# MobilityFirst/gigapaxos

Measured on AMD Instinct MI355X. Metric: decided_ops_per_sec, higher is better.
Workload: dtype int32; 1 GPU; BASELINE config #3: 1000000 Paxos groups x 3 replicas per GPU, synthetic shuffled accept-reply stream; step = propose_batch(G) + accept_reply_batch(K*G votes), inputs resident in HBM; groups_per_gpu=1000000, groups_total=1000000, replicas=3, rounds_seeded_individually=96, ordered_proposals_promise=True, ordered_batches_mask=1, parallelism=groups sharded across GPUs, no collective on the decide path

## Files before the change

gigapaxos_amd/csrc/gpx_ar16.hip.h:

```cpp
#pragma once
#include "gpx_kernels.hip.h"
#include "gpx_tiles.hip.h"

struct __attribute__((aligned(16))) Vote16 {
  int32_t idx, slot, maxcp;
  uint32_t meta;
};
#define V16_LG_MASK 0x3fffu
#define V16_ESC 0x4000u
#define V16_MAX_SHIFT 10
#define GPX_TL_BUCKET_DYN_MAX (152 * 1024)

struct Stage16 {
  int32_t* base;
  int64_t n;
  __host__ __device__ __forceinline__ int32_t* gidx() const { return base; }
  __host__ __device__ __forceinline__ int32_t* slot() const { return base + n; }
  __host__ __device__ __forceinline__ int32_t* bnum() const { return base + 2 * n; }
  __host__ __device__ __forceinline__ int32_t* bcoord() const { return base + 3 * n; }
  __host__ __device__ __forceinline__ int32_t* median() const { return base + 4 * n; }
  __host__ __device__ __forceinline__ uint8_t* kind() const { return (uint8_t*)(base + 5 * n); }
};
struct VoteCols {
  const int32_t *bnum, *bcoord, *acceptor;
  const int32_t *slot, *maxcp;
};
struct PlaceCols {
  int32_t *gidx, *slot, *bnum, *bcoord, *median;
  uint8_t* kind;
  int32_t div;
  uint32_t mul;
  __device__ __forceinline__ int32_t quot(int32_t x) const { return div == 1 ? x : (int32_t)__umulhi((uint32_t)x, mul); }
};
#define GPX_IP_LEARN_WORD 8

__device__ __forceinline__ void put_vote16(const DevScratch& X, int32_t* lds, int32_t G, int32_t mask,
                                           int32_t b0n, int32_t b0c, int64_t i, int32_t g, int32_t slot,
                                           int32_t acc, int32_t maxcp, int32_t bn, int32_t bc) {
  if ((uint32_t)(g - X.g_base) >= (uint32_t)(X.g_end - X.g_base)) return;
  (void)G;
  const int32_t pos = bucket_take(lds, (g - X.g_base) >> X.shift);
  const bool esc = bn != b0n || bc != b0c || (uint32_t)acc > 0xffffu;
  Vote16 v;
  v.idx = (int32_t)i;
  v.slot = slot;
  v.maxcp = maxcp;
  v.meta = (uint32_t)(g & mask) | (esc ? V16_ESC : ((uint32_t)acc << 16));
  ((Vote16*)X.rec)[pos] = v;
}

template <bool VEC>
__global__ __launch_bounds__(GPX_FBLOCK) void k_scatter_ar16(
    int32_t n, int32_t ntiles, int32_t G, DevScratch X, const int32_t* __restrict__ gidx,
    const int32_t* __restrict__ bnum, const int32_t* __restrict__ bcoord,
    const int32_t* __restrict__ slot, const int32_t* __restrict__ acceptor,
    const int32_t* __restrict__ max_cp) {
  extern __shared__ int32_t lds[];
  const int32_t tile = tile_of_block(ntiles);
  if (tile >= ntiles) return;
  if (X.gate && *X.unsorted != X.epoch) return;
  const int32_t b0n = bnum[0], b0c = bcoord[0];
  scatter_init(X, tile, lds);
  const int64_t base = (int64_t)tile * GPX_TILE;
  const int32_t mask = X.gb - 1;
  if (VEC) {
#pragma unroll
    for (int j = 0; j < GPX_TILE_VECS; j++) {
      const int64_t i0 = base + (int64_t)(j * GPX_FBLOCK + threadIdx.x) * 4;
      if (i0 + 3 < n) {
        const I4 g4 = *(const I4*)(gidx + i0), s4 = *(const I4*)(slot + i0);
        const I4 a4 = *(const I4*)(acceptor + i0), m4 = *(const I4*)(max_cp + i0);
        const I4 n4 = *(const I4*)(bnum + i0), c4 = *(const I4*)(bcoord + i0);
        put_vote16(X, lds, G, mask, b0n, b0c, i0 + 0, g4.x, s4.x, a4.x, m4.x, n4.x, c4.x);
        put_vote16(X, lds, G, mask, b0n, b0c, i0 + 1, g4.y, s4.y, a4.y, m4.y, n4.y, c4.y);
        put_vote16(X, lds, G, mask, b0n, b0c, i0 + 2, g4.z, s4.z, a4.z, m4.z, n4.z, c4.z);
        put_vote16(X, lds, G, mask, b0n, b0c, i0 + 3, g4.w, s4.w, a4.w, m4.w, n4.w, c4.w);
      } else {
        for (int q = 0; q < 4; q++) {
          const int64_t i = i0 + q;
          if (i < n)
            put_vote16(X, lds, G, mask, b0n, b0c, i, gidx[i], slot[i], acceptor[i], max_cp[i], bnum[i],
                       bcoord[i]);
        }
      }
    }
  } else {
#pragma unroll
    for (int j = 0; j < GPX_TILE_ITEMS; j++) {
      const int64_t i = base + j * GPX_FBLOCK + threadIdx.x;
      if (i < n)
        put_vote16(X, lds, G, mask, b0n, b0c, i, gidx[i], slot[i], acceptor[i], max_cp[i], bnum[i],
                   bcoord[i]);
    }
  }
// ... 261 lines not shown
        have = true;
        el = el && sl == s0;
      }
      if (have) {
        const int32_t d = jsub(P.next, s0);
        el = el && d >= 1 && d <= S.W;
      }
    }
    fast = __all(el);
  }
  if (fast) {
    if (OP == B16_AR) {
      const int32_t G = S.G, k = (int32_t)GF_K(P.gf);
      int32_t mem[KMAX], ns[KMAX];
#pragma unroll
      for (int j = 0; j < KMAX; j++) {
        mem[j] = (j < k) ? P.mem[j] : 0;
        ns[j] = (j < k) ? P.ns[j] : 0;
      }
      const int64_t off = (int64_t)(s0 & (S.W - 1)) * G + g;
      const uint32_t e0 = (P.have_pe && s0 == jsub(P.next, 1)) ? P.pe : S.p_ring[off];
      uint32_t e = e0;
      int32_t pcount = P.pcount;
      bool ns_dirty = false;
      auto vote = [&](int32_t i, uint32_t p, int32_t acc, int32_t maxcp) {
        int32_t midx = -1;
#pragma unroll
        for (int q = 0; q < KMAX; q++) {
          if (q < k && mem[q] == acc) {
            midx = q;
            if (ns[q] < maxcp) {
              ns[q] = maxcp;
              ns_dirty = true;
            }
          }
        }
        if (e & PR_PRESENT) {
          if (midx >= 0) e |= (1u << midx);
          if (__popc(e & 0xffffu) > k / 2) {
            slotA[p] = s0;
            cpA[p] = median_minus<KMAX>(ns, k);
            metaA[p] = (uint32_t)GPX_D_DECISION;
            it.omask |= 1u << i;
            it.nout++;
            e = 0;
            pcount--;
          }
        }
      };
      if (!__any(esc)) {
        for (int32_t i = 0; i < nvote; i++) {
          const uint32_t p = (uint32_t)start + (uint32_t)pstride * (uint32_t)((it.order >> (4 * i)) & 15ull);
          vote(i, p, (int32_t)(metaA[p] >> 16), cpA[p]);
        }
      } else {
        for (int32_t i = 0; i < nvote; i++) {
          if ((skip >> i) & 1u) continue;
          const uint32_t p = (uint32_t)start + (uint32_t)pstride * (uint32_t)((it.order >> (4 * i)) & 15ull);
          const uint32_t meta = metaA[p];
          vote(i, p, (meta & V16_ESC) ? in.acceptor[idxA[p]] : (int32_t)(meta >> 16), cpA[p]);
        }
      }
      if (e != e0) S.p_ring[off] = e;
      if (ns_dirty) {
#pragma unroll
        for (int q = 0; q < KMAX; q++)
          if (q < k) S.node_slots[(int64_t)q * G + g] = ns[q];
      }
      if (pcount != P.pcount) S.c_pcount[g] = pcount;
    }
  } else {
    replay(it);
  }
}

struct TileLds {
  int32_t* pre;
  uint16_t* st;
};
#define GPX_TILE_LDS_DECL(TILES_)                                   \
  __shared__ int32_t s_pre_[(TILES_) ? GPX_TL_MAXWG + 1 : 1];       \
  __shared__ uint16_t s_st_[(TILES_) ? GPX_TL_MAXWG : 1];           \
  const TileLds TL{s_pre_, s_st_}
template <int OP, int KMAX, bool TILES = false>
__device__ __forceinline__ void bucket16_body(const DevState& S, const DevScratch& X, const Stage16& O, const VoteCols& in,
                                              const AcceptOut& R, uint8_t* __restrict__ status, const TileLds& TL,
                                              const TileArea& A = TileArea{}, int32_t b_in = -1,
                                              const PlaceCols& IP = PlaceCols{}) {
  extern __shared__ __attribute__((aligned(16))) int32_t lds[];
  constexpr bool AC = OP != B16_AR;
  if ((AC || X.gate) && *X.unsorted != X.epoch) return;
  int32_t b = b_in >= 0 ? b_in : (int32_t)blockIdx.x;
  if (TILES && A.xcd_rows && b_in < 0) {
    b = tile_of_block(X.nbk);
    if (b >= X.nbk) return;
  }
  const int32_t gb = X.gb;
  const int32_t l = (int32_t)threadIdx.x;
  int32_t boff, nb;
  int32_t* const s_pre = TL.pre;
  uint16_t* const s_st = TL.st;
  if (TILES) TL_STAMP(4096 + b, 0);
  if (TILES) {
    const unsigned long long* r0 = (const unsigned long long*)A.off + (uint32_t)(b >> 2) * (uint32_t)A.nwg_pad;
    const unsigned long long* r1 = (const unsigned long long*)A.off + (uint32_t)((b + 1) >> 2) * (uint32_t)A.nwg_pad;
    const int32_t per = (A.nwg + gb - 1) >> X.shift;
    int32_t cw[4], ssum = 0, csum = 0;
#pragma unroll
    for (int q = 0; q < 4; q++) {
      const int32_t w = l * per + q;
      cw[q] = 0;
      if (q < per && w < A.nwg) {
        const unsigned long long e0 = r0[w];
        const unsigned long long e1 = ((b & 3) == 3) ? r1[w] : e0;
        const uint16_t o0 = (uint16_t)(e0 >> (16 * (b & 3))), o1 = (uint16_t)(e1 >> (16 * ((b + 1) & 3)));
        const int32_t st = (int32_t)(o0 & 0x7fffu);
        cw[q] = (int32_t)(o1 & 0x7fffu) - st;
        s_st[w] = o0;
        ssum += st;
        csum += cw[q];
      }
    }
    int32_t ex = block_exscan_and_sum_rt(csum, ssum, &nb, &boff);
#pragma unroll
    for (int q = 0; q < 4; q++) {
      const int32_t w = l * per + q;
      if (q < per && w < A.nwg) {
        s_pre[w] = ex;
        ex += cw[q];
      }
    }
    if (l == 0) {
      s_pre[A.nwg] = nb;
      X.bucket_off[b] = boff;
      if (nb == 0) X.bucket_nout[b] = 0;
    }
  } else {
    boff = X.bucket_off[b];
    nb = X.bucket_off[b + 1] - boff;
    if (threadIdx.x == 0) {
      X.bucket_tot[b] = 0;
      if (nb == 0) X.bucket_nout[b] = 0;
    }
  }
  if (nb == 0) return;
  const int32_t g = X.g_base + (b << X.shift) + l;
#ifdef GPX_B16_NOPRELOAD
  const bool pre = false;
#else
  const bool pre = !AC && 2 * nb >= gb;
#endif
  CoordPre<KMAX> P;
  P.have_pe = false;
  P.my_bnum = P.my_bcoord = 0;
  if (pre && g < X.g_end) coord_preload<KMAX>(S, g, P);
  const int32_t L = X.lds_recs;
  int32_t* lcnt = lds;
  int32_t* lcur = lds + gb;
  int32_t* idxA = lds + 2 * gb;
  int32_t* slotA = idxA + L;
  int32_t* cpA = slotA + L;
  uint32_t* metaA = (uint32_t*)(cpA + L);
  const bool in_lds = nb <= L;
  Vote16* recG = (Vote16*)X.rec + boff;
  unsigned long long* keysG = X.perm + boff;
  lcnt[l] = 0;
  const int32_t slot0 = TILES ? A.ref[0] : 0;
  const int32_t ref_bn = TILES ? A.ref[1] : in.bnum[0], ref_bc = TILES ? A.ref[2] : in.bcoord[0];
  int32_t ip_pb = 0, ip_span = -1;
  if (TILES && !AC && IP.div) {
    ip_pb = IP.quot(boff);
    ip_span = IP.quot(boff + nb) - ip_pb;
  }
  int32_t srch = 0;
  if (TILES)
    while ((1 << srch) < A.nwg) srch++;
  auto tile_find = [&](int32_t j) -> int32_t {
    int32_t lo = 0, hi = A.nwg;
    for (int32_t t = 0; t < srch; t++) {
      const int32_t mid = (lo + hi) >> 1;
      const bool up = s_pre[mid] <= j;
      lo = up ? mid : lo;
      hi = up ? hi : mid;
    }
    return lo;
  };
  auto tile_adv = [&](int32_t j, int32_t lo) -> int32_t {
    while (s_pre[lo + 1] <= j) lo++;
    return lo;
  };
  auto tile_pos = [&](int32_t j, int32_t lo, uint32_t* wide) -> uint32_t {
    const uint32_t st = s_st[lo];
    *wide = st & TL_WIDE;
    return __umul24((uint32_t)lo, (uint32_t)A.tile) + (st & 0x7fffu) + (uint32_t)(j - s_pre[lo]);
  };
  auto tile_exp = [&](const Vote8 raw, uint32_t p, uint32_t wide, int32_t lo) -> Vote16 {
    const I4 x = tile_expand(raw, wide ? A.ext + p : (const int2*)nullptr, lo, A.tile, slot0, in.slot, in.maxcp);
    Vote16 v;
    v.idx = x.x, v.slot = x.y, v.maxcp = x.z, v.meta = (uint32_t)x.w;
    return v;
  };
  auto tile_at = [&](int32_t j, int32_t lo) -> Vote16 {
    uint32_t wide;
    const uint32_t p = tile_pos(j, lo, &wide);
    return tile_exp(A.recs[p], p, wide, lo);
  };
  auto tile_rec = [&](int32_t j) -> Vote16 { return tile_at(j, tile_find(j)); };
  if (TILES) __syncthreads();
  if (TILES) TL_STAMP(4096 + b, 1);
#ifdef GPX_ABL_STOP
  if (TILES && GPX_ABL_STOP == 1) return;
#endif
  if (TILES && !in_lds) {
    for (int32_t j = l; j < nb; j += gb) recG[j] = tile_rec(j);
    __threadfence_block();
  }
  __syncthreads();
  Vote16 r0, r1, r2, r3;
  r0.meta = r1.meta = r2.meta = r3.meta = 0;
  r0.idx = r1.idx = r2.idx = r3.idx = 0;
  r0.slot = r1.slot = r2.slot = r3.slot = 0;
  r0.maxcp = r1.maxcp = r2.maxcp = r3.maxcp = 0;
  const bool from_tiles = TILES && in_lds;
  const int32_t pl = from_tiles ? (nb + gb - 1) >> X.shift : 0;
  const int32_t jb = from_tiles ? l * pl : l, jstep = from_tiles ? 1 : gb;
  const int32_t jend = from_tiles ? min(jb + pl, nb) : nb;
  const bool v0 = jb < jend, v1 = jb + jstep < jend, v2 = jb + 2 * jstep < jend, v3 = jb + 3 * jstep < jend;
  int32_t lo3 = 0;
  if (from_tiles) {
    int32_t l0 = 0, l1 = 0, l2 = 0;
    uint32_t p0 = 0, p1 = 0, p2 = 0, p3 = 0, w0 = 0, w1 = 0, w2 = 0, w3 = 0;
    Vote8 q0{}, q1{}, q2{}, q3{};
    if (v0) lo3 = l0 = tile_find(jb), p0 = tile_pos(jb, l0, &w0), q0 = A.recs[p0];
    if (v1) lo3 = l1 = tile_adv(jb + 1, l0), p1 = tile_pos(jb + 1, l1, &w1), q1 = A.recs[p1];
    if (v2) lo3 = l2 = tile_adv(jb + 2, l1), p2 = tile_pos(jb + 2, l2, &w2), q2 = A.recs[p2];
    if (v3) lo3 = tile_adv(jb + 3, l2), p3 = tile_pos(jb + 3, lo3, &w3), q3 = A.recs[p3];
    if (v0) r0 = tile_exp(q0, p0, w0, l0);
    if (v1) r1 = tile_exp(q1, p1, w1, l1);
    if (v2) r2 = tile_exp(q2, p2, w2, l2);
    if (v3) r3 = tile_exp(q3, p3, w3, lo3);
  } else {
    if (v0) r0 = recG[jb];
    if (v1) r1 = recG[jb + jstep];
    if (v2) r2 = recG[jb + 2 * jstep];
    if (v3) r3 = recG[jb + 3 * jstep];
  }
  const int32_t tail0 = jb + 4 * jstep;
  auto for_tail = [&](auto&& f) {
    if (from_tiles) {
      int32_t lo = lo3;
      for (int32_t j = tail0; j < jend; j++) {
        lo = tile_adv(j, lo);
        f(tile_at(j, lo));
      }
    } else {
      for (int32_t j = tail0; j < jend; j += jstep) f(recG[j]);
    }
  };
  constexpr int KSLOT = KMAX <= 4 ? 4 : 8;
  bool slotted = false;
  if (TILES && !AC && in_lds && KSLOT * gb <= L) {
    bool over = false;
    auto put_row = [&](const Vote16& v) {
      const int32_t lg = (int32_t)(v.meta & V16_LG_MASK);
      const int32_t t = atomicAdd(&lcnt[lg], 1);
      if (t < KSLOT) {
        const int32_t p = t * gb + lg;
        idxA[p] = v.idx;
        slotA[p] = v.slot;
        cpA[p] = v.maxcp;
        metaA[p] = v.meta;
      } else {
        over = true;
      }
    };
    if (v0) put_row(r0);
    if (v1) put_row(r1);
    if (v2) put_row(r2);
    if (v3) put_row(r3);
    for_tail([&](const Vote16& v) { put_row(v); });
    slotted = !__syncthreads_or(over);
    if (!slotted) {
      lcnt[l] = 0;
      __syncthreads();
    }
  }
  int32_t c, start, any_long = 0;
  if (slotted) {
    c = lcnt[l];
    start = l;
    if (TILES) TL_STAMP(4096 + b, 3);
#ifdef GPX_ABL_STOP
    if (TILES && GPX_ABL_STOP == 2) return;
#endif
    if (pre && g < X.g_end) coord_preload_ring<KMAX>(S, g, P);
  } else {
  {
    if (v0) atomicAdd(&lcnt[r0.meta & V16_LG_MASK], 1);
    if (v1) atomicAdd(&lcnt[r1.meta & V16_LG_MASK], 1);
    if (v2) atomicAdd(&lcnt[r2.meta & V16_LG_MASK], 1);
// ... 132 lines not shown
    it.cur = 0;
    if (live) ar16_replay_group<OP, KMAX>(S, X, g, it, P, in, R, status, idxA, slotA, cpA, metaA, start, pstride, c);
    nout = it.nout;
    omask = it.omask;
    if (TILES) TL_STAMP(4096 + b, 4);
#ifdef GPX_ABL_STOP
    if (TILES && GPX_ABL_STOP == 3) return;
#endif
    int32_t tout;
    const int32_t ex = block_exscan_rt(nout, &tout);
    const int32_t pb = in_place(tout);
    for (int32_t q = 0; q < nout; q++) {
      int32_t sl, md, kd;
      it.output(q, &sl, &md, &kd, &omask);
      put((int64_t)boff + ex + q, sl, md, kd);
      if (pb >= 0) put_in_place(pb + ex + q, sl, md, kd);
    }
    if (l == 0) X.bucket_nout[b] = tout;
    if (TILES) TL_STAMP(4096 + b, 5);
  } else {
    VoteIter<false, AC> it;
    it.idxA = idxA;
    it.slotA = slotA;
    it.cpA = cpA;
    it.metaA = metaA;
    it.recG = recG;
    it.keys = keysG + start;
    it.in = in;
    it.b0n = ref_bn;
    it.b0c = ref_bc;
    it.start = start;
    it.stride = 1;
    it.c = c;
    it.done = 0;
    it.nout = 0;
    it.nib = false;
    it.order = 0;
    it.omask = 0;
    it.cur = 0;
    if (live) replay(it);
    nout = it.nout;
    int32_t tout;
    const int32_t ex = block_exscan_rt(nout, &tout);
    const int32_t pb = in_place(tout);
    for (int32_t q = 0; q < nout; q++) {
      int32_t sl, md, kd;
      it.output(q, &sl, &md, &kd, &omask);
      put((int64_t)boff + ex + q, sl, md, kd);
      if (pb >= 0) put_in_place(pb + ex + q, sl, md, kd);
    }
    if (l == 0) X.bucket_nout[b] = tout;
  }
}

template <int OP, int KMAX>
__global__ __launch_bounds__(1024) GPX_AR16_ATTR void k_bucket16(DevState S, DevScratch X, Stage16 O, VoteCols in,
                                                   AcceptOut R, uint8_t* __restrict__ status) {
  GPX_TILE_LDS_DECL(false);
  bucket16_body<OP, KMAX>(S, X, O, in, R, status, TL);
}
struct TilesKernArgs {
  DevState S;
  DevScratch X;
  Stage16 O;
  VoteCols in;
  uint8_t* status;
  TileArea A;
  PlaceCols IP;
};
static_assert(alignof(DevState) == 8 && alignof(DevScratch) == 8 && alignof(Stage16) == 8 && alignof(VoteCols) == 8 &&
                  alignof(TileArea) == 8 && alignof(PlaceCols) == 8,
              "kernarg layout");
static_assert(sizeof(DevState) % 8 == 0 && sizeof(DevScratch) % 8 == 0 && sizeof(Stage16) % 8 == 0 && sizeof(VoteCols) % 8 == 0 &&
                  sizeof(TileArea) % 8 == 0 && sizeof(PlaceCols) % 8 == 0,
              "kernarg layout");
#ifndef GPX_LAZY
#define GPX_LAZY 7
#endif
template <bool LAZY, class T>
__device__ __forceinline__ const T& lazy_pick(const T& from_kernarg, const T& by_value) {
  if constexpr (LAZY) return from_kernarg;
  else return by_value;
}
#define GPX_TILES_KERNEL_BODY(KM)                                                                                          \
  GPX_TILE_LDS_DECL(true);                                                                                                 \
  const TilesKernArgs* ka = (const TilesKernArgs*)__builtin_amdgcn_kernarg_segment_ptr();                                  \
  bucket16_body<B16_AR, KM, true>(lazy_pick<(GPX_LAZY & 16) != 0>(ka->S, S), lazy_pick<(GPX_LAZY & 2) != 0>(ka->X, X), O,  \
                                  lazy_pick<(GPX_LAZY & 1) != 0>(ka->in, in), AcceptOut{},                                 \
                                  (GPX_LAZY & 8) ? ka->status : status, TL, lazy_pick<(GPX_LAZY & 32) != 0>(ka->A, A), -1, \
                                  lazy_pick<(GPX_LAZY & 4) != 0>(ka->IP, IP))
template <int KMAX>
__global__ __launch_bounds__(1024) GPX_AR16_ATTR void k_bucket_ar16_tiles(DevState S, DevScratch X, Stage16 O, VoteCols in,
                                                                         uint8_t* __restrict__ status, TileArea A, PlaceCols IP) {
  GPX_TILES_KERNEL_BODY(KMAX);
}
#ifndef GPX_K4_WAVES
#define GPX_K4_WAVES 6
#endif
__global__ __launch_bounds__(1024) __attribute__((amdgpu_waves_per_eu(GPX_K4_WAVES, 8))) void k_bucket_ar16_tiles_k4(
    DevState S, DevScratch X, Stage16 O, VoteCols in, uint8_t* __restrict__ status, TileArea A, PlaceCols IP) {
  GPX_TILES_KERNEL_BODY(4);
}
__global__ __launch_bounds__(1024) __attribute__((amdgpu_waves_per_eu(6, 8))) void k_bucket_ar16_tiles_k5(
    DevState S, DevScratch X, Stage16 O, VoteCols in, uint8_t* __restrict__ status, TileArea A, PlaceCols IP) {
  GPX_TILES_KERNEL_BODY(5);
}
__global__ __launch_bounds__(1024) __attribute__((amdgpu_waves_per_eu(6, 8))) void k_bucket_ar16_k5(
    DevState S, DevScratch X, Stage16 O, VoteCols in, AcceptOut R, uint8_t* __restrict__ status) {
  GPX_TILE_LDS_DECL(false);
  bucket16_body<B16_AR, 5>(S, X, O, in, R, status, TL);
}

__global__ __launch_bounds__(GPX_BLOCK) void k_emit_dec16(
    DevScratch X, Stage16 O, int32_t* __restrict__ d_gidx, int32_t* __restrict__ d_slot,
    int32_t* __restrict__ d_bnum, int32_t* __restrict__ d_bcoord, int32_t* __restrict__ d_median,
    uint8_t* __restrict__ d_kind, int32_t* total_out, unsigned long long* acc, const int32_t* base_in,
    int32_t* chain_out, int32_t* in_place = nullptr, int32_t nvotes = 0, const int32_t* __restrict__ c_bnum = nullptr,
    const int32_t* __restrict__ c_bcoord = nullptr) {
  if (X.gate && *X.unsorted != X.epoch) return;
  const bool placed = in_place && in_place[3] != (int32_t)X.epoch;
  if (placed && blockIdx.x != gridDim.x - 1) return;
  const int32_t base0 = base_in ? *base_in : 0;
  const int32_t b = blockIdx.x;
  int32_t before = 0;
  for (int32_t t = threadIdx.x; t < b; t += GPX_BLOCK) before += X.bucket_nout[t];
  int32_t pre;
  block_exscan(before, &pre);
  const int32_t out0 = base0 + pre;
  if (b == (int32_t)gridDim.x - 1 && threadIdx.x == 0) {
    const int32_t tot = pre + X.bucket_nout[b];
    if (total_out) *total_out = base0 + tot;
    if (chain_out) *chain_out = base0 + tot;
    if (acc) atomicAdd(acc, (unsigned long long)tot);
    if (in_place && !placed && tot > 0 && nvotes % tot == 0 && nvotes / tot <= 64 && X.xabort)
      __hip_atomic_store(X.xabort + GPX_IP_LEARN_WORD, (uint32_t)(nvotes / tot), __ATOMIC_RELAXED, __HIP_MEMORY_SCOPE_SYSTEM);
    if (in_place) in_place[placed ? 5 : 6]++;
  }
  if (placed) return;
  const int32_t nd = X.bucket_nout[blockIdx.x];
  const int64_t src = X.bucket_off[blockIdx.x];
  if (threadIdx.x == 0) X.bucket_tot[blockIdx.x] = 0;
  for (int32_t t = threadIdx.x; t < nd; t += GPX_BLOCK) {
    const int32_t g = O.gidx()[src + t];
    d_gidx[out0 + t] = g;
    d_slot[out0 + t] = O.slot()[src + t];
    d_bnum[out0 + t] = c_bnum ? c_bnum[g] : O.bnum()[src + t];
    d_bcoord[out0 + t] = c_bnum ? c_bcoord[g] : O.bcoord()[src + t];
    d_median[out0 + t] = O.median()[src + t];
    d_kind[out0 + t] = O.kind()[src + t];
  }
}

__global__ __launch_bounds__(GPX_BLOCK) void k_emit_runs16(DevScratch X, Stage16 O, int32_t* __restrict__ x_gidx,
                                                          int32_t* __restrict__ x_first,
                                                          int32_t* __restrict__ x_count, int32_t* total_out) {
  if (*X.unsorted != X.epoch) return;
  const int32_t out0 = emit_base(X, total_out, nullptr);
  const int32_t nd = X.bucket_nout[blockIdx.x];
  const int64_t src = X.bucket_off[blockIdx.x];
  for (int32_t t = threadIdx.x; t < nd; t += GPX_BLOCK) {
    x_gidx[out0 + t] = O.gidx()[src + t];
    x_first[out0 + t] = O.slot()[src + t];
    x_count[out0 + t] = O.median()[src + t];
  }
}

__global__ __launch_bounds__(GPX_BLOCK) void k_unpack_replies(DevScratch X, int32_t n, const I4* __restrict__ rows,
                                                             int32_t* __restrict__ r_bnum,
                                                             int32_t* __restrict__ r_bcoord,
                                                             int32_t* __restrict__ r_maxcp,
                                                             uint8_t* __restrict__ r_flags) {
  if (*X.unsorted != X.epoch) return;
  const int32_t i = blockIdx.x * GPX_BLOCK + threadIdx.x;
  if (i >= n) return;
  const I4 r = rows[i];
  r_bnum[i] = r.x;
  r_bcoord[i] = r.y;
  r_maxcp[i] = r.z;
  r_flags[i] = (uint8_t)r.w;
}
```

gigapaxos_amd/csrc/gpx_kernels.hip.h:

```cpp
#pragma once
#include <hip/hip_runtime.h>
#include <stdint.h>

#include "../../include/gpx.h"

#ifdef GPX_SAR_TRACE
__device__ unsigned long long* g_sar_trace = nullptr;
#define SAR_STAMP(wg, k)                                                                             \
  do {                                                                                               \
    if (threadIdx.x == 0 && g_sar_trace) g_sar_trace[(size_t)(wg) * 16 + (k)] = wall_clock64();        \
  } while (0)
#else
#define SAR_STAMP(wg, k) do { } while (0)
#endif

#ifdef GPX_TL_TRACE
__device__ unsigned long long* g_tl_trace = nullptr;
#define TL_TRACE_ROWS 8192
#define TL_STAMP(row, k)                                                                             \
  do {                                                                                               \
    if (threadIdx.x == 0 && g_tl_trace) g_tl_trace[(size_t)(row) * 8 + (k)] = wall_clock64();          \
  } while (0)
#define TL_CLOCK(row, k)  \
  do {                                                                                               \
// ... 405 lines not shown
    const uint8_t* __restrict__ flags, int32_t* __restrict__ r_bnum, int32_t* __restrict__ r_bcoord,
    int32_t* __restrict__ r_maxcp, uint8_t* __restrict__ r_flags, int32_t only_unsorted) {
  extern __shared__ int32_t lds[];
  const int32_t tile = tile_of_block(ntiles);
  if (tile >= ntiles) return;
  if (only_unsorted && *X.unsorted != X.epoch) return;
  scatter_init(X, tile, lds);
  const int64_t base = (int64_t)tile * GPX_TILE;
  const int32_t mask = X.gb - 1;
  auto one = [&](int64_t i, int32_t g, int32_t a, int32_t b, int32_t c, int32_t bn, int32_t bc) {
    put_rec(X, lds, G, mask, i, g, a, b, c, bn, bc);
    if ((uint32_t)g >= (uint32_t)G && r_bnum) {
      r_bnum[i] = 0;
      r_bcoord[i] = 0;
      r_maxcp[i] = 0;
      r_flags[i] = 0;
    }
  };
  if (VEC) {
#pragma unroll
    for (int j = 0; j < GPX_TILE_VECS; j++) {
      const int64_t i0 = base + (int64_t)(j * GPX_FBLOCK + threadIdx.x) * 4;
      if (i0 + 3 < n) {
        const I4 g4 = *(const I4*)(gidx + i0), s4 = *(const I4*)(slot + i0);
        const I4 m4 = *(const I4*)(median_cp + i0);
        const I4 n4 = *(const I4*)(bnum + i0), c4 = *(const I4*)(bcoord + i0);
        const uint32_t f4 = flags ? *(const uint32_t*)(flags + i0) : 0u;
        one(i0 + 0, g4.x, s4.x, m4.x, (int32_t)(f4 & 0xffu), n4.x, c4.x);
        one(i0 + 1, g4.y, s4.y, m4.y, (int32_t)((f4 >> 8) & 0xffu), n4.y, c4.y);
        one(i0 + 2, g4.z, s4.z, m4.z, (int32_t)((f4 >> 16) & 0xffu), n4.z, c4.z);
        one(i0 + 3, g4.w, s4.w, m4.w, (int32_t)(f4 >> 24), n4.w, c4.w);
      } else {
        for (int q = 0; q < 4; q++) {
          const int64_t i = i0 + q;
          if (i < n) one(i, gidx[i], slot[i], median_cp[i], flags ? (int32_t)flags[i] : 0, bnum[i], bcoord[i]);
        }
      }
    }
  } else {
#pragma unroll
    for (int j = 0; j < GPX_TILE_ITEMS; j++) {
      const int64_t i = base + j * GPX_FBLOCK + threadIdx.x;
      if (i < n) one(i, gidx[i], slot[i], median_cp[i], flags ? (int32_t)flags[i] : 0, bnum[i], bcoord[i]);
    }
  }
}

__global__ __launch_bounds__(GPX_FBLOCK) void k_scatter_pr(
    int32_t n, int32_t ntiles, int32_t G, DevScratch X, const int32_t* __restrict__ gidx,
    const uint8_t* __restrict__ is_stop, int32_t* __restrict__ o_slot, int32_t* __restrict__ o_bnum,
    int32_t* __restrict__ o_bcoord, int32_t* __restrict__ o_median) {
  extern __shared__ int32_t lds[];
  const int32_t tile = tile_of_block(ntiles);
  if (tile >= ntiles) return;
  if (*X.unsorted != X.epoch) return;
  scatter_init(X, tile, lds);
  const int64_t base = (int64_t)tile * GPX_TILE;
  const int32_t mask = X.gb - 1;
#pragma unroll
  for (int j = 0; j < GPX_TILE_ITEMS; j++) {
    const int64_t i = base + j * GPX_FBLOCK + threadIdx.x;
    if (i < n) {
      const int32_t g = gidx[i];
      put_rec(X, lds, G, mask, i, g, is_stop ? (int32_t)(is_stop[i] & 1) : 0, 0, 0, 0, 0);
      if ((uint32_t)g >= (uint32_t)G) {
        o_slot[i] = 0;
        o_bnum[i] = 0;
        o_bcoord[i] = 0;
        o_median[i] = 0;
      }
    }
  }
}


__device__ __forceinline__ void cmpxchg_asc(unsigned long long* a, uint32_t lo, uint32_t hi) {
  unsigned long long x = a[lo], y = a[hi];
  if (x > y) {
    a[lo] = y;
    a[hi] = x;
  }
}

__device__ void sort_long_segment(unsigned long long* a, uint32_t c) {
  uint32_t p2 = 1;
  while (p2 < c) p2 <<= 1;
  for (uint32_t k = 2; k <= p2; k <<= 1) {
    for (uint32_t t = threadIdx.x; t < c; t += blockDim.x) {
      const uint32_t q = t ^ (k - 1);
      if (q > t && q < c) cmpxchg_asc(a, t, q);
    }
    __syncthreads();
    for (uint32_t j = k >> 2; j > 0; j >>= 1) {
      for (uint32_t t = threadIdx.x; t < c; t += blockDim.x) {
        const uint32_t q = t ^ j;
        if (q > t && q < c) cmpxchg_asc(a, t, q);
      }
      __syncthreads();
    }
  }
}

__device__ __forceinline__ int32_t block_exscan_rt(int32_t v, int32_t* total) {
  __shared__ int32_t wsum[16];
  const int lane = threadIdx.x & 63, wid = threadIdx.x >> 6;
  const int nw = (int)(blockDim.x >> 6);
  const int32_t x = wave_incscan(v);
  if (lane == 63) wsum[wid] = x;
  __syncthreads();
  const int32_t ps = wave_incscan(lane < nw ? wsum[lane] : 0);
  const int32_t tot = __shfl(ps, nw - 1, 64);
  const int32_t base = __shfl(ps, wid > 0 ? wid - 1 : 0, 64);
  __syncthreads();
  *total = tot;
  return (wid > 0 ? base : 0) + x - v;
}

__device__ __forceinline__ int32_t block_exscan_and_sum_rt(int32_t v, int32_t u, int32_t* vtotal, int32_t* utotal) {
  __shared__ int32_t wsum2[32];
  const int lane = threadIdx.x & 63, wid = threadIdx.x >> 6;
  const int nw = (int)(blockDim.x >> 6);
  const int32_t x = wave_incscan(v), y = wave_incscan(u);
  if (lane == 63) {
    wsum2[wid] = x;
    wsum2[16 + wid] = y;
  }
  __syncthreads();
  const int32_t ps = wave_incscan(lane < nw ? wsum2[lane] : 0);
  const int32_t pu = wave_incscan(lane < nw ? wsum2[16 + lane] : 0);
  const int32_t tot = __shfl(ps, nw - 1, 64);
  const int32_t base = __shfl(ps, wid > 0 ? wid - 1 : 0, 64);
  *utotal = __shfl(pu, nw - 1, 64);
  __syncthreads();
  *vtotal = tot;
  return (wid > 0 ? base : 0) + x - v;
}

struct BucketView {
  int32_t* pay;
  int32_t rs, fs;
  unsigned long long* keys;
  int32_t* lcnt;
  int32_t* loff;
};

#define GPX_PAY_WORDS 5
#define GPX_BUCKET_ITEMS 8
#define GPX_BUCKET_LDS_BYTES(gb, lds_recs) \
  ((size_t)(gb) * 8 + (size_t)(lds_recs) * (8 + 4 * GPX_PAY_WORDS))

template <class F>
__device__ __forceinline__ bool bucket_prepare(const DevScratch& X, int32_t* lds, BucketView* bv,
                                               F after_a) {
  const int32_t b = blockIdx.x;
  const int32_t boff = X.bucket_off[b];
  const int32_t nb = X.bucket_off[b + 1] - boff;
  if (threadIdx.x == 0) {
    X.bucket_tot[b] = 0;
    if (nb == 0) X.bucket_nout[b] = 0;
  }
  if (nb == 0) return false;
  const int32_t gb = X.gb;
  const int32_t nt = (int32_t)blockDim.x;
  int32_t* lcnt = lds;
  int32_t* loff = lds + gb;
  unsigned long long* keysL = (unsigned long long*)(lds + 2 * gb);
  int32_t* payL = (int32_t*)(keysL + X.lds_recs);
// ... 1599 lines not shown
```

gigapaxos_amd/csrc/gpx_tiles.hip.h:

```cpp
#pragma once
#include "gpx_kernels.hip.h"

__host__ __device__ __forceinline__ int32_t tl_cnt_words(int32_t nbk, int32_t nt) {
  const int32_t per = (nbk + 1 + nt - 1) / nt;
  return nt * (per <= 4 ? 4 : 8);
}
#ifndef GPX_TL_MAXWG
#define GPX_TL_MAXWG 1024
#endif
struct __attribute__((aligned(8))) Vote8 {
  uint32_t a;
  uint32_t b;
};
#define V8_ESC_S 0x40000000u
#define V8_ESC_B 0x80000000u
#define TL_WIDE 0x8000u
struct TileArea {
  Vote8* recs;
  int2* ext;
  uint16_t* off;
  int32_t* ref;
  int32_t nwg, nwg_pad, tile;
  int32_t xcd_rows;
};
// ... 25 lines not shown
  int32_t cx = __shfl(x, 0, 64), cy = __shfl(y, 0, 64);
  const int32_t fx = cx, fy = cy;
  for (int t = 0; t < 4; t++) {
    const unsigned long long same = __ballot(x == cx && y == cy) & act;
    if (2 * __popcll(same) > __popcll(act)) {
      *ox = cx, *oy = cy;
      return;
    }
    tried |= same;
    const unsigned long long rest = act & ~tried;
    if (!rest) break;
    const int nl = __ffsll((long long)rest) - 1;
    cx = __shfl(x, nl, 64), cy = __shfl(y, nl, 64);
  }
  (void)lane;
  *ox = fx, *oy = fy;
}

__device__ __forceinline__ void store16_through(I4* dst, const I4 v) {
#ifdef GPX_NO_SC1_STORES
  *dst = v;
#else
  gpx_i32x4 x;
  x.x = v.x, x.y = v.y, x.z = v.z, x.w = v.w;
  asm volatile("global_store_dwordx4 %0, %1, off sc1" ::"v"(dst), "v"(x) : "memory");
#endif
}

template <bool FULL, int NTB = 0>
__device__ __forceinline__ I4 tiles_load4(const int32_t* __restrict__ col, int64_t i0, int32_t n, int32_t fill) {
  if (FULL) return stream_load16<NTB>((const I4*)(col + i0));
  I4 r;
  r.x = i0 + 0 < n ? stream_load4<NTB>(col + i0 + 0) : fill;
  r.y = i0 + 1 < n ? stream_load4<NTB>(col + i0 + 1) : fill;
  r.z = i0 + 2 < n ? stream_load4<NTB>(col + i0 + 2) : fill;
  r.w = i0 + 3 < n ? stream_load4<NTB>(col + i0 + 3) : fill;
  return r;
}

template <int NT>
__device__ __forceinline__ int32_t tl_block_exscan(int32_t v, int32_t* total, int32_t* wsum) {
  const int lane = threadIdx.x & 63, wid = threadIdx.x >> 6;
  const int32_t x = wave_incscan(v);
  if (lane == 63) wsum[wid] = x;
  __syncthreads();
  const int32_t ps = wave_incscan(lane < NT / 64 ? wsum[lane] : 0);
  *total = __shfl(ps, NT / 64 - 1, 64);
  const int32_t base = __shfl(ps, wid > 0 ? wid - 1 : 0, 64);
  return (wid > 0 ? base : 0) + x - v;
}
struct __attribute__((aligned(8))) Off4 {
  uint16_t h[4];
};
template <int NT, int P>
__device__ __forceinline__ int32_t tl_publish_starts(int32_t* cnt, int32_t* s_wsum, const TileArea& A, int32_t w, int32_t nbk,
                                                     uint32_t wf) {
  static_assert(P % 4 == 0, "whole entries of A.off");
  const int32_t bq = (int32_t)threadIdx.x * P;
  int32_t v[P], s = 0;
#pragma unroll
  for (int q = 0; q < P; q++) {
    v[q] = cnt[bq + q];
    s += v[q];
  }
  int32_t tot;
  int32_t ex = tl_block_exscan<NT>(s, &tot, s_wsum);
#pragma unroll
  for (int q4 = 0; q4 < P; q4 += 4) {
    Off4 o;
#pragma unroll
    for (int q = 0; q < 4; q++) {
      cnt[bq + q4 + q] = ex;
      o.h[q] = (uint16_t)((uint32_t)ex | wf);
      ex += v[q4 + q];
    }
#ifdef GPX_TL_TRACE
    if (A.xcd_rows & 2) continue;
#endif
    if (bq + q4 <= nbk) ((Off4*)A.off)[(uint32_t)((bq + q4) >> 2) * (uint32_t)A.nwg_pad + (uint32_t)w] = o;
  }
  return tot;
}

#define TL_RK_MASK 0x3fffu
template <int NT, int R4, bool FULL>
__device__ __forceinline__ void scatter_tile(int32_t n, int32_t G, const DevScratch& X, const TileArea& A, int32_t w,
                                             const int32_t* __restrict__ gidx, const int32_t* __restrict__ bnum,
                                             const int32_t* __restrict__ bcoord, const int32_t* __restrict__ slot,
                                             const int32_t* __restrict__ acceptor, const int32_t* __restrict__ max_cp,
                                             uint8_t* __restrict__ status, int32_t* cnt, Vote8* recs, const int32_t* s_ref,
                                             int32_t* s_nesc, int32_t* s_wsum) {
  constexpr int T = NT * 4 * R4;
  constexpr int U = (R4 == 2) ? 2 : 1;
  const int32_t nbk = X.nbk;
  const int32_t slot0 = s_ref[0], b0n = s_ref[1], b0c = s_ref[2];
  const int32_t shift = X.shift, mask = X.gb - 1;
  const int64_t t0 = (int64_t)w * T + (int64_t)threadIdx.x * 4;
  int32_t gg[R4 * 4];
  uint32_t bw[R4 * 4], rk[R4 * 4];
  int32_t bad = 0, nesc = 0;
  int32_t chain = 0;
#pragma unroll
  for (int k0 = 0; k0 < R4; k0 += U) {
    I4 g4[U], s4[U], a4[U], m4[U], n4[U], c4[U];
#pragma unroll
    for (int u = 0; u < U; u++) {
      const int64_t i0 = t0 + (int64_t)(k0 + u) * NT * 4 + chain;
      g4[u] = tiles_load4<FULL, GPX_NT_VOTES>(gidx, i0, n, -1);
      s4[u] = tiles_load4<FULL, GPX_NT_VOTES>(slot, i0, n, 0);
      a4[u] = tiles_load4<FULL, GPX_NT_VOTES>(acceptor, i0, n, 0);
      m4[u] = tiles_load4<FULL, GPX_NT_VOTES>(max_cp, i0, n, 0);
      n4[u] = tiles_load4<FULL, GPX_NT_VOTES>(bnum, i0, n, 0);
      c4[u] = tiles_load4<FULL, GPX_NT_VOTES>(bcoord, i0, n, 0);
    }
#pragma unroll
    for (int u = 0; u < U; u++) {
      const int k = k0 + u;
      const int64_t i0 = t0 + (int64_t)k * NT * 4;
      const int32_t g_[4] = {g4[u].x, g4[u].y, g4[u].z, g4[u].w}, ss[4] = {s4[u].x, s4[u].y, s4[u].z, s4[u].w};
      const int32_t aa[4] = {a4[u].x, a4[u].y, a4[u].z, a4[u].w}, mm[4] = {m4[u].x, m4[u].y, m4[u].z, m4[u].w};
      const int32_t nn[4] = {n4[u].x, n4[u].y, n4[u].z, n4[u].w}, cc[4] = {c4[u].x, c4[u].y, c4[u].z, c4[u].w};
      uint32_t stw = 0;
      int32_t av[4];
#pragma unroll
      for (int q = 0; q < 4; q++) {
        const bool in_batch = FULL || i0 + q < n;
        const bool ok = in_batch && (uint32_t)g_[q] < (uint32_t)G;
        av[q] = atomicAdd(&cnt[ok ? (g_[q] >> shift) : 0], ok ? 1 : 0);
        if (in_batch && !ok) {
          bad++;
          stw |= (uint32_t)GPX_S_NOGROUP << (8 * q);
        }
      }
#pragma unroll
      for (int q = 0; q < 4; q++) {
        const int e = k * 4 + q;
        const bool ok = (FULL || i0 + q < n) && (uint32_t)g_[q] < (uint32_t)G;
        const uint32_t dslot = (uint32_t)(ss[q] - slot0 + 128), dcp = (uint32_t)(ss[q] - 1 - mm[q] + 128);
        const bool es = dslot > 255u || dcp > 255u;
        const bool eb = nn[q] != b0n || cc[q] != b0c || (uint32_t)aa[q] > 0xffffu;
        gg[e] = ok ? g_[q] : -1;
        bw[e] = (es ? 0u : (dslot | (dcp << 8))) | (eb ? 0u : ((uint32_t)aa[q] << 16));
        rk[e] = (uint32_t)av[q] | (es ? V8_ESC_S : 0u) | (eb ? V8_ESC_B : 0u);
        nesc += (ok && es) ? 1 : 0;
      }
#ifdef GPX_TL_TRACE
      if (A.xcd_rows & 4) continue;
#endif
      if (status) {
        if (FULL) {
          stream_store4<GPX_NT_PREFILL>((uint32_t*)(status + i0), stw);
        } else {
          for (int q = 0; q < 4; q++)
            if (i0 + q < n) stream_store1<GPX_NT_PREFILL>(status + i0 + q, (uint8_t)((stw >> (8 * q)) & 0xffu));
        }
      }
    }
    chain = (int32_t)rk[(k0 + U) * 4 - 1];
    asm volatile("v_and_b32 %0, 0, %0" : "+v"(chain));
  }
  if (bad) atomicAdd(&X.counters[2], (unsigned long long)bad);
  if (nesc) atomicAdd(s_nesc, nesc);
  if (w == 0 && threadIdx.x == 0) atomicAdd(&X.counters[0], (unsigned long long)n);
  __syncthreads();
  TL_STAMP(w, 1);
#pragma unroll
  for (int e = 0; e < R4 * 4; e++) asm volatile("" : "+v"(gg[e]), "+v"(rk[e]), "+v"(bw[e]));
  const bool wide = *s_nesc * 32 > T;
  const uint32_t wf = wide ? TL_WIDE : 0u;
  const int32_t per = (nbk + 1 + NT - 1) / NT;
  int32_t tot;
  if (per <= 4) tot = tl_publish_starts<NT, 4>(cnt, s_wsum, A, w, nbk, wf);
  else tot = tl_publish_starts<NT, 8>(cnt, s_wsum, A, w, nbk, wf);
  (void)per;
  __syncthreads();
  TL_STAMP(w, 2);
  const uint32_t keep = wide ? V8_ESC_B : (V8_ESC_S | V8_ESC_B);
#pragma unroll
  for (int k = 0; k < R4; k++) {
    int32_t pos[4];
#pragma unroll
    for (int q = 0; q < 4; q++) pos[q] = cnt[max(gg[k * 4 + q], 0) >> shift];
#pragma unroll
    for (int q = 0; q < 4; q++) {
      const int e = k * 4 + q;
      const int32_t g = gg[e];
      Vote8 r;
      r.a = (uint32_t)(k * NT * 4 + (int32_t)threadIdx.x * 4 + q) | ((uint32_t)(g & mask) << 14) | (rk[e] & keep);
      r.b = bw[e];
      if (g >= 0) recs[pos[q] + (int32_t)(rk[e] & TL_RK_MASK)] = r;
    }
  }
  __syncthreads();
  TL_STAMP(w, 3);
  {
    const I4* src = (const I4*)recs;
    I4* dst = (I4*)(A.recs + (int64_t)w * T);
    const int32_t nv = (tot + 1) >> 1;
    int32_t i = (int32_t)threadIdx.x;
    for (; i + NT < nv; i += 2 * NT) {
      const I4 x = src[i], y = src[i + NT];
      store16_through(dst + i, x);
      store16_through(dst + i + NT, y);
    }
    if (i < nv) store16_through(dst + i, src[i]);
  }
  if (wide) {
    __syncthreads();
    int2* ext = (int2*)recs;
#pragma unroll
    for (int k = 0; k < R4; k++) {
      const int64_t i0 = t0 + (int64_t)k * NT * 4;
      const I4 s4 = tiles_load4<FULL>(slot, i0, n, 0), m4 = tiles_load4<FULL>(max_cp, i0, n, 0);
      const int32_t ss[4] = {s4.x, s4.y, s4.z, s4.w}, mm[4] = {m4.x, m4.y, m4.z, m4.w};
#pragma unroll
      for (int q = 0; q < 4; q++) {
        const int e = k * 4 + q;
        if (gg[e] >= 0) ext[cnt[gg[e] >> shift] + (int32_t)(rk[e] & TL_RK_MASK)] = make_int2(ss[q], mm[q]);
      }
    }
    __syncthreads();
    const I4* src = (const I4*)recs;
    I4* dst = (I4*)(A.ext + (int64_t)w * T);
    const int32_t nv = (tot + 1) >> 1;
    for (int32_t i = (int32_t)threadIdx.x; i < nv; i += NT) store16_through(dst + i, src[i]);
  }
  TL_STAMP(w, 4);
  TL_CLOCK(w, 7);
}

template <int NT, int R4>
__global__ __launch_bounds__(NT) void k_scatter_tiles(int32_t n, int32_t G, DevScratch X, TileArea A,
                                                      const int32_t* __restrict__ gidx, const int32_t* __restrict__ bnum,
                                                      const int32_t* __restrict__ bcoord, const int32_t* __restrict__ slot,
                                                      const int32_t* __restrict__ acceptor,
                                                      const int32_t* __restrict__ max_cp, uint8_t* __restrict__ status) {
  extern __shared__ __attribute__((aligned(16))) int32_t lds[];
  constexpr int T = NT * 4 * R4;
  static_assert(T <= 16384, "14 bits of tile offset, 15 bits of run start");
  const int32_t nbk = X.nbk;
  Vote8* recs = (Vote8*)lds;
  int32_t* cnt = lds + 2 * T;
  int32_t* s_ref = cnt + tl_cnt_words(nbk, NT);
  int32_t* s_nesc_p = s_ref + 4;
  int32_t* s_wsum = s_ref + 8;
  const int32_t w = tile_of_block(A.nwg);
  if (w >= A.nwg) return;
  if (X.gate && *X.unsorted != X.epoch) return;
  TL_STAMP(w, 0);
  TL_CLOCK(w, 6);
  for (int32_t b = threadIdx.x; b < tl_cnt_words(nbk, NT); b += NT) cnt[b] = 0;
  if (threadIdx.x < 64) {
    const int32_t m = min(n, 64), i = min((int32_t)threadIdx.x, m - 1);
    int32_t rb, rc, rs, dummy;
    wave_majority2(bnum[i], bcoord[i], m, &rb, &rc);
    wave_majority2(slot[i], 0, m, &rs, &dummy);
    if (threadIdx.x == 0) {
      s_ref[0] = rs, s_ref[1] = rb, s_ref[2] = rc;
      *s_nesc_p = 0;
      if (w == 0) A.ref[0] = rs, A.ref[1] = rb, A.ref[2] = rc;
    }
  }
  __syncthreads();
  if ((int64_t)(w + 1) * T <= n && !((uintptr_t)status & 3))
    scatter_tile<NT, R4, true>(n, G, X, A, w, gidx, bnum, bcoord, slot, acceptor, max_cp, status, cnt, recs, s_ref, s_nesc_p, s_wsum);
  else
    scatter_tile<NT, R4, false>(n, G, X, A, w, gidx, bnum, bcoord, slot, acceptor, max_cp, status, cnt, recs, s_ref, s_nesc_p, s_wsum);
}
#define GPX_TL_LDS_BYTES(nbk, T, NT) ((size_t)tl_cnt_words(nbk, NT) * 4 + (size_t)(T) * sizeof(Vote8) + 128)
```

Baseline: 12.98 billion decisions/s.

## Add two-word fast path for K4 tile buckets and issue scatter loads early

Adds a specialized fast path in the K<=4 tiled accept-reply bucket kernel. Each bucket's votes are packed into per-group two-word rows in LDS, sorted with a small network, and applied directly when every group decides exactly one slot, with a fallback to the general path otherwise. The tile scatter kernel now issues its first round of vote loads before the prologue (counter zeroing and majority reference), so memory latency overlaps that setup. Both are enabled by default through macros. The cost is more registers and LDS pressure, plus an extra block-wide reduction, in the K4 kernel.

```diff
diff --git a/gigapaxos_amd/csrc/gpx_ar16.hip.h b/gigapaxos_amd/csrc/gpx_ar16.hip.h
--- a/gigapaxos_amd/csrc/gpx_ar16.hip.h
+++ b/gigapaxos_amd/csrc/gpx_ar16.hip.h
@@ -10,6 +10,9 @@
 #define V16_ESC 0x4000u
 #define V16_MAX_SHIFT 10
 #define GPX_TL_BUCKET_DYN_MAX (152 * 1024)
+#ifndef GPX_AR16_TWO_WORD
+#define GPX_AR16_TWO_WORD 1
+#endif
 
 struct Stage16 {
   int32_t* base;
@@ -437,7 +440,7 @@
   __shared__ int32_t s_pre_[(TILES_) ? GPX_TL_MAXWG + 1 : 1];       \
   __shared__ uint16_t s_st_[(TILES_) ? GPX_TL_MAXWG : 1];           \
   const TileLds TL{s_pre_, s_st_}
-template <int OP, int KMAX, bool TILES = false>
+template <int OP, int KMAX, bool TILES = false, bool TWO = false>
 __device__ __forceinline__ void bucket16_body(const DevState& S, const DevScratch& X, const Stage16& O, const VoteCols& in,
                                               const AcceptOut& R, uint8_t* __restrict__ status, const TileLds& TL,
                                               const TileArea& A = TileArea{}, int32_t b_in = -1,
@@ -455,6 +458,8 @@
   int32_t boff, nb;
   int32_t* const s_pre = TL.pre;
   uint16_t* const s_st = TL.st;
+  constexpr bool TW = TILES && !AC && TWO;
+  bool wide_run = false;
   if (TILES) TL_STAMP(4096 + b, 0);
   if (TILES) {
     const unsigned long long* r0 = (const unsigned long long*)A.off + (uint32_t)(b >> 2) * (uint32_t)A.nwg_pad;
@@ -471,6 +476,7 @@
         const uint16_t o0 = (uint16_t)(e0 >> (16 * (b & 3))), o1 = (uint16_t)(e1 >> (16 * ((b + 1) & 3)));
         const int32_t st = (int32_t)(o0 & 0x7fffu);
         cw[q] = (int32_t)(o1 & 0x7fffu) - st;
+        wide_run = wide_run || ((o0 & TL_WIDE) && cw[q] > 0);
         s_st[w] = o0;
         ssum += st;
         csum += cw[q];
@@ -561,7 +567,11 @@
     return tile_exp(A.recs[p], p, wide, lo);
   };
   auto tile_rec = [&](int32_t j) -> Vote16 { return tile_at(j, tile_find(j)); };
-  if (TILES) __syncthreads();
+  bool any_wide = false;
+  if (TILES) {
+    if (TW) any_wide = __syncthreads_or(wide_run);
+    else __syncthreads();
+  }
   if (TILES) TL_STAMP(4096 + b, 1);
 #ifdef GPX_ABL_STOP
   if (TILES && GPX_ABL_STOP == 1) return;
@@ -571,6 +581,155 @@
     __threadfence_block();
   }
   __syncthreads();
+  if constexpr (TW) {
+    constexpr int KS = 4;
+    static_assert(KMAX <= 4, "eight rows of two words beside the K = 5 state do not fit the kernel's registers");
+    const bool full_bucket = X.g_base + ((b + 1) << X.shift) <= X.g_end;
+    if (in_lds && KS * gb <= L && nb >= gb && nb <= KS * gb && full_bucket && !any_wide && pre) {
+      uint2* rows = (uint2*)idxA;
+      const int32_t pl = (nb + gb - 1) >> X.shift;
+      const int32_t jb = l * pl, jend = min(jb + pl, nb);
+      bool bad = false;
+      auto put2 = [&](const Vote8 q, int32_t lo) {
+        const int32_t lg = (int32_t)((q.a >> 14) & 0x3ffu);
+        const int32_t t = atomicAdd(&lcnt[lg], 1);
+        if (t < KS && !(q.a & V8_ESC_S))
+          rows[t * gb + lg] = make_uint2(((((uint32_t)lo << 14) | (q.a & 0x3fffu)) << 1) | (q.a >> 31), q.b);
+        else
+          bad = true;
+      };
+      {
+        const bool v0 = jb < jend, v1 = jb + 1 < jend, v2 = jb + 2 < jend, v3 = jb + 3 < jend;
+        int32_t l0 = 0, l1 = 0, l2 = 0, l3 = 0;
+        uint32_t wd;
+        Vote8 q0{}, q1{}, q2{}, q3{};
+        if (v0) l3 = l0 = tile_find(jb), q0 = A.recs[tile_pos(jb, l0, &wd)];
+        if (v1) l3 = l1 = tile_adv(jb + 1, l0), q1 = A.recs[tile_pos(jb + 1, l1, &wd)];
+        if (v2) l3 = l2 = tile_adv(jb + 2, l1), q2 = A.recs[tile_pos(jb + 2, l2, &wd)];
+        if (v3) l3 = tile_adv(jb + 3, l2), q3 = A.recs[tile_pos(jb + 3, l3, &wd)];
+        if (v0) put2(q0, l0);
+        if (v1) put2(q1, l1);
+        if (v2) put2(q2, l2);
+        if (v3) put2(q3, l3);
+      }
+      __syncthreads();
+      TL_STAMP(4096 + b, 3);
+      coord_preload_ring<KMAX>(S, g, P);
+      const int32_t c = lcnt[l];
+      uint32_t ky0, ky1, ky2, ky3, bw0, bw1, bw2, bw3;
+#define GPX_ROW(t)                               \
+  {                                              \
+    const uint2 r_ = rows[t * gb + l];           \
+    ky##t = t < c ? r_.x : 0xffffffffu;          \
+    bw##t = r_.y;                                \
+  }
+      GPX_ROW(0) GPX_ROW(1) GPX_ROW(2) GPX_ROW(3)
+#undef GPX_ROW
+      bool ok = !bad && c >= 1 &&
+                (P.gf & (GF_EXISTS | GF_STOPPED | GF_HASCOORD | GF_PREPARING)) == (GF_EXISTS | GF_HASCOORD) &&
+                ref_bn == P.my_bnum && ref_bc == P.my_bcoord;
+#define GPX_CHK(t) ok = ok && (t >= c || (!(ky##t & 1u) && ((bw##t ^ bw0) & 255u) == 0));
+      GPX_CHK(0) GPX_CHK(1) GPX_CHK(2) GPX_CHK(3)
+#undef GPX_CHK
+      const int32_t s0 = slot0 + (int32_t)(bw0 & 255u) - 128;
+      {
+        const int32_t d = jsub(P.next, s0);
+        ok = ok && d >= 1 && d <= S.W;
+      }
+#define GPX_CX(i, j)                                                                     \
+  {                                                                                      \
+    const bool sw_ = ky##i > ky##j;                                                      \
+    const uint32_t lo_ = min(ky##i, ky##j), hi_ = max(ky##i, ky##j);                     \
+    const uint32_t bl_ = sw_ ? bw##j : bw##i, bh_ = sw_ ? bw##i : bw##j;                 \
+    ky##i = lo_, ky##j = hi_, bw##i = bl_, bw##j = bh_;                                  \
+  }
+      GPX_CX(0, 1) GPX_CX(2, 3) GPX_CX(0, 2) GPX_CX(1, 3) GPX_CX(1, 2)
+#undef GPX_CX
+      const int32_t G = S.G, k = (int32_t)GF_K(P.gf);
+      int32_t mem[KMAX], ns[KMAX];
+#pragma unroll
+      for (int j = 0; j < KMAX; j++) {
+        mem[j] = (j < k) ? P.mem[j] : 0;
+        ns[j] = (j < k) ? P.ns[j] : 0;
+      }
+      const int64_t off = (int64_t)(s0 & (S.W - 1)) * G + g;
+      uint32_t e0 = 0;
+      if (ok) e0 = (s0 == P.pe_slot) ? P.pe : S.p_ring[off];
+      uint32_t e = e0;
+      int32_t pcount = P.pcount, ndec = 0, md = 0;
+      bool ns_dirty = false;
+      auto vote = [&](bool on, uint32_t w_) {
+        if (!on) return;
+        const int32_t acc = (int32_t)(w_ >> 16), maxcp = s0 - 1 - ((int32_t)((w_ >> 8) & 255u) - 128);
+        int32_t midx = -1;
+#pragma unroll
+        for (int q = 0; q < KMAX; q++) {
+          if (q < k && mem[q] == acc) {
+            midx = q;
+            if (ns[q] < maxcp) {
+              ns[q] = maxcp;
+              ns_dirty = true;
+            }
+          }
+        }
+        if (e & PR_PRESENT) {
+          if (midx >= 0) e |= (1u << midx);
+          if (__popc(e & 0xffffu) > k / 2) {
+            md = median_minus<KMAX>(ns, k);
+            ndec++;
+            e = 0;
+            pcount--;
+          }
+        }
+      };
+      vote(0 < c, bw0), vote(1 < c, bw1), vote(2 < c, bw2), vote(3 < c, bw3);
+      ok = ok && ndec == 1;
+      if (!__syncthreads_or(!ok)) {
+        TL_STAMP(4096 + b, 4);
+        S.p_ring[off] = e;
+        if (ns_dirty) {
+#pragma unroll
+          for (int q = 0; q < KMAX; q++)
+            if (q < k) S.node_slots[(int64_t)q * G + g] = ns[q];
+        }
+        S.c_pcount[g] = pcount;
+        const int64_t o = (int64_t)boff + l;
+        if ((GPX_NT_STREAMS & GPX_NT_STAGE) && IP.div) {
+          stream_store4<GPX_NT_STAGE>(&O.gidx()[o], g);
+          stream_store4<GPX_NT_STAGE>(&O.slot()[o], s0);
+          stream_store4<GPX_NT_STAGE>(&O.median()[o], md);
+          stream_store1<GPX_NT_STAGE>(&O.kind()[o], (uint8_t)GPX_D_DECISION);
+        } else {
+          O.gidx()[o] = g;
+          O.slot()[o] = s0;
+          O.median()[o] = md;
+          if (!IP.div) {
+            O.bnum()[o] = P.my_bnum;
+            O.bcoord()[o] = P.my_bcoord;
+          }
+          O.kind()[o] = (uint8_t)GPX_D_DECISION;
+        }
+        if (IP.div) {
+          if (gb == ip_span) {
+            const int32_t q = ip_pb + l;
+            stream_store4<GPX_NT_PLACE>(&IP.gidx[q], g);
+            stream_store4<GPX_NT_PLACE>(&IP.slot[q], s0);
+            stream_store4<GPX_NT_PLACE>(&IP.median[q], md);
+            stream_store4<GPX_NT_PLACE>(&IP.bnum[q], P.my_bnum);
+            stream_store4<GPX_NT_PLACE>(&IP.bcoord[q], P.my_bcoord);
+            stream_store1<GPX_NT_PLACE>(&IP.kind[q], (uint8_t)GPX_D_DECISION);
+          } else if (l == 0) {
+            A.ref[3] = (int32_t)X.epoch;
+          }
+        }
+        if (l == 0) X.bucket_nout[b] = gb;
+        TL_STAMP(4096 + b, 5);
+        return;
+      }
+      lcnt[l] = 0;
+      __syncthreads();
+    }
+  }
   Vote16 r0, r1, r2, r3;
   r0.meta = r1.meta = r2.meta = r3.meta = 0;
   r0.idx = r1.idx = r2.idx = r3.idx = 0;
@@ -869,28 +1028,30 @@
   if constexpr (LAZY) return from_kernarg;
   else return by_value;
 }
-#define GPX_TILES_KERNEL_BODY(KM)                                                                                          \
-  GPX_TILE_LDS_DECL(true);                                                                                                 \
-  const TilesKernArgs* ka = (const TilesKernArgs*)__builtin_amdgcn_kernarg_segment_ptr();                                  \
-  bucket16_body<B16_AR, KM, true>(lazy_pick<(GPX_LAZY & 16) != 0>(ka->S, S), lazy_pick<(GPX_LAZY & 2) != 0>(ka->X, X), O,  \
-                                  lazy_pick<(GPX_LAZY & 1) != 0>(ka->in, in), AcceptOut{},                                 \
-                                  (GPX_LAZY & 8) ? ka->status : status, TL, lazy_pick<(GPX_LAZY & 32) != 0>(ka->A, A), -1, \
-                                  lazy_pick<(GPX_LAZY & 4) != 0>(ka->IP, IP))
+#define GPX_TILES_KERNEL_BODY(KM, TWO_)                                                                                         \
+  GPX_TILE_LDS_DECL(true);                                                                                                      \
+  constexpr bool two_ = (TWO_) && GPX_AR16_TWO_WORD != 0;                                                                       \
+  const TilesKernArgs* ka = (const TilesKernArgs*)__builtin_amdgcn_kernarg_segment_ptr();                                       \
+  bucket16_body<B16_AR, KM, true, two_>(lazy_pick<(GPX_LAZY & 16) != 0>(ka->S, S), lazy_pick<(GPX_LAZY & 2) != 0>(ka->X, X), O, \
+                                        lazy_pick<(GPX_LAZY & 1) != 0>(ka->in, in), AcceptOut{},                                \
+                                        (GPX_LAZY & 8) ? ka->status : status, TL,                                               \
+                                        lazy_pick<(GPX_LAZY & 32) != 0 || two_>(ka->A, A), -1,                                  \
+                                        lazy_pick<(GPX_LAZY & 4) != 0>(ka->IP, IP))
 template <int KMAX>
 __global__ __launch_bounds__(1024) GPX_AR16_ATTR void k_bucket_ar16_tiles(DevState S, DevScratch X, Stage16 O, VoteCols in,
                                                                          uint8_t* __restrict__ status, TileArea A, PlaceCols IP) {
-  GPX_TILES_KERNEL_BODY(KMAX);
+  GPX_TILES_KERNEL_BODY(KMAX, false);
 }
 #ifndef GPX_K4_WAVES
 #define GPX_K4_WAVES 6
 #endif
 __global__ __launch_bounds__(1024) __attribute__((amdgpu_waves_per_eu(GPX_K4_WAVES, 8))) void k_bucket_ar16_tiles_k4(
     DevState S, DevScratch X, Stage16 O, VoteCols in, uint8_t* __restrict__ status, TileArea A, PlaceCols IP) {
-  GPX_TILES_KERNEL_BODY(4);
+  GPX_TILES_KERNEL_BODY(4, true);
 }
 __global__ __launch_bounds__(1024) __attribute__((amdgpu_waves_per_eu(6, 8))) void k_bucket_ar16_tiles_k5(
     DevState S, DevScratch X, Stage16 O, VoteCols in, uint8_t* __restrict__ status, TileArea A, PlaceCols IP) {
-  GPX_TILES_KERNEL_BODY(5);
+  GPX_TILES_KERNEL_BODY(5, false);
 }
 __global__ __launch_bounds__(1024) __attribute__((amdgpu_waves_per_eu(6, 8))) void k_bucket_ar16_k5(
     DevState S, DevScratch X, Stage16 O, VoteCols in, AcceptOut R, uint8_t* __restrict__ status) {
diff --git a/gigapaxos_amd/csrc/gpx_kernels.hip.h b/gigapaxos_amd/csrc/gpx_kernels.hip.h
--- a/gigapaxos_amd/csrc/gpx_kernels.hip.h
+++ b/gigapaxos_amd/csrc/gpx_kernels.hip.h
@@ -511,7 +511,7 @@
   }
 }
 
-__device__ void sort_long_segment(unsigned long long* a, uint32_t c) {
+__device__ __forceinline__ void sort_long_segment(unsigned long long* a, uint32_t c) {
   uint32_t p2 = 1;
   while (p2 < c) p2 <<= 1;
   for (uint32_t k = 2; k <= p2; k <<= 1) {
diff --git a/gigapaxos_amd/csrc/gpx_tiles.hip.h b/gigapaxos_amd/csrc/gpx_tiles.hip.h
--- a/gigapaxos_amd/csrc/gpx_tiles.hip.h
+++ b/gigapaxos_amd/csrc/gpx_tiles.hip.h
@@ -131,27 +131,42 @@
   return tot;
 }
 
+#ifndef GPX_TL_EARLY_LOADS
+#define GPX_TL_EARLY_LOADS 1
+#endif
+template <int NT>
+__device__ __forceinline__ void tl_prologue(int32_t n, int32_t nbk, const TileArea& A, int32_t w, const int32_t* __restrict__ bnum,
+                                            const int32_t* __restrict__ bcoord, const int32_t* __restrict__ slot, int32_t* cnt,
+                                            int32_t* s_ref, int32_t* s_nesc) {
+  for (int32_t b = threadIdx.x; b < tl_cnt_words(nbk, NT); b += NT) cnt[b] = 0;
+  if (threadIdx.x < 64) {
+    const int32_t m = min(n, 64), i = min((int32_t)threadIdx.x, m - 1);
+    int32_t rb, rc, rs, dummy;
+    wave_majority2(bnum[i], bcoord[i], m, &rb, &rc);
+    wave_majority2(slot[i], 0, m, &rs, &dummy);
+    if (threadIdx.x == 0) {
+      s_ref[0] = rs, s_ref[1] = rb, s_ref[2] = rc;
+      *s_nesc = 0;
+      if (w == 0) A.ref[0] = rs, A.ref[1] = rb, A.ref[2] = rc;
+    }
+  }
+}
+
 #define TL_RK_MASK 0x3fffu
 template <int NT, int R4, bool FULL>
 __device__ __forceinline__ void scatter_tile(int32_t n, int32_t G, const DevScratch& X, const TileArea& A, int32_t w,
                                              const int32_t* __restrict__ gidx, const int32_t* __restrict__ bnum,
                                              const int32_t* __restrict__ bcoord, const int32_t* __restrict__ slot,
                                              const int32_t* __restrict__ acceptor, const int32_t* __restrict__ max_cp,
-                                             uint8_t* __restrict__ status, int32_t* cnt, Vote8* recs, const int32_t* s_ref,
+                                             uint8_t* __restrict__ status, int32_t* cnt, Vote8* recs, int32_t* s_ref,
                                              int32_t* s_nesc, int32_t* s_wsum) {
   constexpr int T = NT * 4 * R4;
   constexpr int U = (R4 == 2) ? 2 : 1;
   const int32_t nbk = X.nbk;
-  const int32_t slot0 = s_ref[0], b0n = s_ref[1], b0c = s_ref[2];
   const int32_t shift = X.shift, mask = X.gb - 1;
   const int64_t t0 = (int64_t)w * T + (int64_t)threadIdx.x * 4;
-  int32_t gg[R4 * 4];
-  uint32_t bw[R4 * 4], rk[R4 * 4];
-  int32_t bad = 0, nesc = 0;
-  int32_t chain = 0;
-#pragma unroll
-  for (int k0 = 0; k0 < R4; k0 += U) {
-    I4 g4[U], s4[U], a4[U], m4[U], n4[U], c4[U];
+  I4 g4[U], s4[U], a4[U], m4[U], n4[U], c4[U];
+  auto load_round = [&](int k0, int32_t chain) {
 #pragma unroll
     for (int u = 0; u < U; u++) {
       const int64_t i0 = t0 + (int64_t)(k0 + u) * NT * 4 + chain;
@@ -162,6 +177,20 @@
       n4[u] = tiles_load4<FULL, GPX_NT_VOTES>(bnum, i0, n, 0);
       c4[u] = tiles_load4<FULL, GPX_NT_VOTES>(bcoord, i0, n, 0);
     }
+  };
+  if (GPX_TL_EARLY_LOADS) {
+    load_round(0, 0);
+    tl_prologue<NT>(n, nbk, A, w, bnum, bcoord, slot, cnt, s_ref, s_nesc);
+    __syncthreads();
+  }
+  const int32_t slot0 = s_ref[0], b0n = s_ref[1], b0c = s_ref[2];
+  int32_t gg[R4 * 4];
+  uint32_t bw[R4 * 4], rk[R4 * 4];
+  int32_t bad = 0, nesc = 0;
+  int32_t chain = 0;
+#pragma unroll
+  for (int k0 = 0; k0 < R4; k0 += U) {
+    if (!GPX_TL_EARLY_LOADS || k0 > 0) load_round(k0, chain);
 #pragma unroll
     for (int u = 0; u < U; u++) {
       const int k = k0 + u;
@@ -298,19 +327,10 @@
   if (X.gate && *X.unsorted != X.epoch) return;
   TL_STAMP(w, 0);
   TL_CLOCK(w, 6);
-  for (int32_t b = threadIdx.x; b < tl_cnt_words(nbk, NT); b += NT) cnt[b] = 0;
-  if (threadIdx.x < 64) {
-    const int32_t m = min(n, 64), i = min((int32_t)threadIdx.x, m - 1);
-    int32_t rb, rc, rs, dummy;
-    wave_majority2(bnum[i], bcoord[i], m, &rb, &rc);
-    wave_majority2(slot[i], 0, m, &rs, &dummy);
-    if (threadIdx.x == 0) {
-      s_ref[0] = rs, s_ref[1] = rb, s_ref[2] = rc;
-      *s_nesc_p = 0;
-      if (w == 0) A.ref[0] = rs, A.ref[1] = rb, A.ref[2] = rc;
-    }
-  }
-  __syncthreads();
+  if (!GPX_TL_EARLY_LOADS) {
+    tl_prologue<NT>(n, nbk, A, w, bnum, bcoord, slot, cnt, s_ref, s_nesc_p);
+    __syncthreads();
+  }
   if ((int64_t)(w + 1) * T <= n && !((uintptr_t)status & 3))
     scatter_tile<NT, R4, true>(n, G, X, A, w, gidx, bnum, bcoord, slot, acceptor, max_cp, status, cnt, recs, s_ref, s_nesc_p, s_wsum);
   else
```

Result: faster. 14.12 billion decisions/s, median of 6 (+8.8%).
